# BioinformaticsArchive/HSA

Hardware: AMD Instinct MI355X
Metric: aligned reads/sec, 100bp synthetic vs hg19-sized 2BWT, at 1/2/4/8 MI355X (higher is better)
Workload: dtype u32

## Files before the change

hsa_amd/csrc/hsa_index.hip:

```cpp
#include <chrono>
#include <cstring>
#include <hip/hip_runtime.h>
#include <rocprim/rocprim.hpp>
#include <stdarg.h>
#include <stdio.h>
#include <stdlib.h>
#include <string.h>

#include "hsa_device.h"
#include "hsa_internal.h"
#include "hsa_trie.h"

static thread_local char g_err[1024] = "";
int g_waves_per_cu = 32;
int g_pool_entries = 0;
int g_batch_k = getenv("HSA_BATCH_K") ? atoi(getenv("HSA_BATCH_K")) : 32;
int g_batch_idle = getenv("HSA_BATCH_IDLE") ? atoi(getenv("HSA_BATCH_IDLE")) : 768;
int g_hit_cap = 64;

void hsa_set_error(const char *fmt, ...)
{
    va_list ap;
    va_start(ap, fmt);
    vsnprintf(g_err, sizeof g_err, fmt, ap);
    va_end(ap);
}

extern "C" const char *hsa_last_error(void) { return g_err; }
extern "C" void hsa_gpu_set_error_text(const char *msg) { hsa_set_error("%s", msg); }

extern "C" int hsa_device_count(void)
{
    int n = 0;
    if (hipGetDeviceCount(&n) != hipSuccess) return 0;
    return n;
}

extern "C" void hsa_free(void *p) { free(p); }

extern "C" int hsa_configure(int waves_per_cu, int pool_entries, int hit_cap)
{
    if (waves_per_cu > 0) g_waves_per_cu = waves_per_cu;
    if (pool_entries > 0) {
        if (pool_entries > 65535) { hsa_set_error("pool_entries > 65535"); return HSA_E_ARG; }
        g_pool_entries = pool_entries;
    } else if (pool_entries < 0) {
        g_pool_entries = 0;
    }
    if (hit_cap > 0) g_hit_cap = hit_cap;
    return 0;
}

static void hsa_log_alloc(const char *what, size_t bytes, std::chrono::steady_clock::time_point t0)
{
    const double ms = std::chrono::duration<double, std::milli>(std::chrono::steady_clock::now() - t0).count();
    if (ms > 5.0 && getenv("HSA_VERBOSE")) fprintf(stderr, "[hsa] %s: hipMalloc of %.2f GB took %.1f ms\n", what, bytes / 1e9, ms);
}

int hsa_realloc_device(void **out, void **old, size_t bytes)
{
    *out = nullptr;
    if (hipMalloc(out, bytes) != hipSuccess) {
        (void)hipGetLastError();
        *out = nullptr;
        (void)hipFree(*old);
        *old = nullptr;
        if (hipMalloc(out, bytes) != hipSuccess) {
            (void)hipGetLastError();
            *out = nullptr;
            hsa_set_error("hipMalloc(%zu) failed", bytes);
            return HSA_E_MEM;
        }
        return 0;
    }
    (void)hipFree(*old);
    *old = nullptr;
    return 0;
}

int hsa_grow(void **p, size_t *cap, size_t need)
{
    if (need <= *cap && *p) return 0;
    size_t n = need + need / 4 + 4096;
    const auto t0 = std::chrono::steady_clock::now();
    void *np = nullptr;
    *cap = 0;
    if (hsa_realloc_device(&np, p, n)) return HSA_E_MEM;
    *p = np;
    *cap = n;
    hsa_log_alloc("buffer", n, t0);
    return 0;
}

void hsa_scratch_free(SearchScratch &s)
{
    (void)hipFree(s.pool); (void)hipFree(s.nxt); (void)hipFree(s.hbuf);
    const size_t lb = s.link_bytes;
    s = SearchScratch();
    s.link_bytes = lb;
}

extern "C" int hsa_index_release_scratch(hsa_index_t *ix)
{
    if (!ix) { hsa_set_error("hsa_index_release_scratch: null handle"); return HSA_E_ARG; }
    (void)hipSetDevice(ix->device);
    HSA_HIP(hipStreamSynchronize(ix->stream));
    hsa_scratch_free(ix->main); hsa_scratch_free(ix->big); hsa_scratch_free(ix->huge);
    void **bufs[] = {&ix->d_pf, &ix->d_pf2, &ix->d_sp, &ix->d_any, &ix->d_any_aux, &ix->d_help, &ix->d_hp, &ix->d_rf,
                     &ix->d_ch, &ix->d_sm};
    size_t *caps[] = {&ix->d_pf_cap, &ix->d_pf2_cap, &ix->d_sp_cap, &ix->d_any_cap, &ix->d_any_aux_cap, &ix->d_help_cap,
                      &ix->d_hp_cap, &ix->d_rf_cap, &ix->d_ch_cap, &ix->d_sm_cap};
    for (int i = 0; i < 10; ++i) {
        if (*bufs[i]) (void)hipFree(*bufs[i]);
        *bufs[i] = nullptr;
        *caps[i] = 0;
    }
    return 0;
}

int hsa_scratch_reserve(SearchScratch &s, size_t lanes, size_t pcap, size_t hcap, size_t link_bytes)
{
    const size_t pe = lanes * pcap, he = lanes * hcap;
    auto fail = [&]() {
        hsa_set_error("scratch allocation failed (lanes %zu, pool %zu, hits %zu)", lanes, pcap, hcap);
        (void)hipGetLastError();
        hsa_scratch_free(s);
        return HSA_E_MEM;
    };
    if (!s.pool || pe > s.pool_entries || link_bytes != s.link_bytes) {
        const size_t npe = pe > s.pool_entries ? pe : s.pool_entries;
        const auto t0 = std::chrono::steady_clock::now();
        void *np = nullptr, *nn = nullptr;
        if (hsa_realloc_device(&np, (void **)&s.pool, npe * sizeof(uint4)) ||
            hsa_realloc_device(&nn, &s.nxt, npe * link_bytes)) {
            (void)hipFree(np);
            return fail();
        }
        s.pool = (uint4 *)np; s.nxt = nn;
        s.pool_entries = npe;
        s.link_bytes = link_bytes;
        hsa_log_alloc("search scratch pool", npe * (sizeof(uint4) + link_bytes), t0);
    }
    if (!s.hbuf || he > s.hit_entries) {
        const size_t nhe = he > s.hit_entries ? he : s.hit_entries;
        const auto t0 = std::chrono::steady_clock::now();
        void *nh = nullptr;
        if (hsa_realloc_device(&nh, (void **)&s.hbuf, nhe * 9 * sizeof(uint32_t))) return fail();
        s.hbuf = (uint32_t *)nh;
        s.hit_entries = nhe;
        hsa_log_alloc("search scratch hits", nhe * 9 * sizeof(uint32_t), t0);
    }
    return 0;
}

__global__ void k_msb_to_lsb(uint32_t *w, size_t n, uint32_t T)
{
    size_t i = (size_t)blockIdx.x * blockDim.x + threadIdx.x;
    if (i >= n) return;
    uint32_t x = w[i];
    x = (x >> 16) | (x << 16);
    x = ((x & 0xFF00FF00u) >> 8) | ((x & 0x00FF00FFu) << 8);
    x = ((x & 0xF0F0F0F0u) >> 4) | ((x & 0x0F0F0F0Fu) << 4);
    x = ((x & 0xCCCCCCCCu) >> 2) | ((x & 0x33333333u) << 2);
    if (i == n - 1 && (T & 15)) x &= (1u << (2 * (T & 15))) - 1u;
    w[i] = x;
}

struct U4 { uint32_t a, b, c, d; };
struct U4Plus {
    __host__ __device__ U4 operator()(const U4 &x, const U4 &y) const
    {
        return U4{x.a + y.a, x.b + y.b, x.c + y.c, x.d + y.d};
    }
};
// ... 704 lines not shown
```

hsa_amd/csrc/hsa_internal.h:

```cpp
#pragma once
#include <hip/hip_runtime.h>
#include <stdint.h>
#include <string>

#include "../../include/hsa_gpu.h"
#include "hsa_device.h"
#include "hsa_sa.h"

void hsa_set_error(const char *fmt, ...);

#define HSA_HIP(call)                                                                       \
    do {                                                                                    \
        hipError_t e_ = (call);                                                             \
        if (e_ != hipSuccess) {                                                             \
            hsa_set_error("%s:%d %s: %s", __FILE__, __LINE__, #call, hipGetErrorString(e_)); \
            return HSA_E_HIP;                                                               \
        }                                                                                   \
    } while (0)

enum : uint32_t {
    CTR_Q_MAIN = 0,
    CTR_HITS = 1,
    CTR_RANK = 2,
    CTR_SECTORS = 3,
    CTR_POPS = 4,
    CTR_ERRORS = 5,
    CTR_Q_FWD = 6,
    CTR_WIDTH_Q = 7,
    CTR_OVF_MAIN = 8,
    CTR_Q_BIG = 9,
    CTR_TRIE = 10,
    CTR_Q_MG = 10,
    CTR_UNFINISHED = 11,
    CTR_OVF_BIG = 12,
    CTR_FWD_Q_ALL = 13,
    CTR_FWD_Q_REF = 14,
    CTR_Q_HUGE = 15,
    CTR_SLOTS = 16
};

struct SearchScratch {
    size_t pool_entries = 0, hit_entries = 0;
    uint4 *pool = nullptr;
    void *nxt = nullptr;
    uint32_t *hbuf = nullptr;
    size_t link_bytes = 2;
};

struct hsa_index {
    int device = 0;
    uint32_t T = 0, isa0 = 0, C[5] = {0, 0, 0, 0, 0};
    uint32_t rT = 0, risa0 = 0, rC[5] = {0, 0, 0, 0, 0};
    uint4 *blk[2] = {nullptr, nullptr};
    void *blk_base[2] = {nullptr, nullptr};
    size_t nblk[2] = {0, 0};
    bool wide = false, is64 = false;
    uint64_t T64 = 0, isa0_64 = 0, C64[5] = {0, 0, 0, 0, 0};
    uint64_t rT64 = 0, risa0_64 = 0, rC64[5] = {0, 0, 0, 0, 0};
    bool any_wrap[2] = {false, false};
    hipStream_t stream = nullptr;
    int n_cu = 0;
    SearchScratch main, big, huge;
    void *d_ovf2 = nullptr; size_t d_ovf2_cap = 0;
    void *d_in = nullptr; size_t d_in_cap = 0;
    void *d_out = nullptr; size_t d_out_cap = 0;
    void *d_wrows = nullptr; size_t d_wrows_cap = 0;
    void *d_ovf = nullptr; size_t d_ovf_cap = 0;
    void *d_seed = nullptr; size_t d_seed_cap = 0;
    void *d_ext = nullptr; size_t d_ext_cap = 0;
    void *d_slices = nullptr; size_t d_slices_cap = 0;
    void *d_any = nullptr; size_t d_any_cap = 0;
    void *d_any_aux = nullptr; size_t d_any_aux_cap = 0;
    void *d_split = nullptr; size_t d_split_cap = 0;
    void *d_help = nullptr; size_t d_help_cap = 0;
    void *d_fwd = nullptr; size_t d_fwd_cap = 0;
    void *d_pf = nullptr; size_t d_pf_cap = 0;
    void *d_pf2 = nullptr; size_t d_pf2_cap = 0;
    void *h_pf = nullptr; size_t h_pf_cap = 0;
    uint32_t *d_sa = nullptr, *d_blocks = nullptr;
// ... 76 lines not shown
```

hsa_amd/csrc/hsa_search_kernels.h:

```cpp
#pragma once
#include <hip/hip_runtime.h>
#include <stdio.h>
#include <stdlib.h>
#include <string.h>

#include <type_traits>

#include "hsa_device.h"
#include "hsa_internal.h"
#include "hsa_trie.h"

#define NIL16 0xFFFFu
#define BLOCK 256
#define MAXB 128
#define MAXS 512

enum : uint32_t { PH_IDLE = 0, PH_POP, PH_EXACT, PH_EXPAND, PH_EXIT, PH_END, PH_WAIT };

struct SearchArgs {
    RankDir fwd, rev;
    uint32_t T;
    uint32_t C[5];
    RankDir64 fwd64, rev64;
    uint64_t T64;
// ... 41 lines not shown
    const int32_t *perm;
    uint32_t okey;
    int32_t *fwd_list;
    unsigned long long *fwd_n;
    uint32_t fwd_only;
    int32_t *rmap;
    uint32_t fr_budget, fr_demand, fr_cap;
    uint32_t *fr_ent;
    uint32_t *fr_tag;
    uint32_t *fr_rq;
    uint32_t *fr_st;
    unsigned long long *fr_q, *fr_p;
    unsigned long long *fr_c;
    const void *stw;
    uint32_t sdc;
};
#define FR_HIT 0x80000000u
#define FR_DONE 0x40000000u
#define FR_EW 8u
#define FR_CH 16u
#define FR_WALK 1024u
#ifndef HSA_HELPERS
#define HSA_HELPERS 1
#endif

typedef const __attribute__((address_space(4))) SearchArgs *ColdArgs;
__device__ __forceinline__ ColdArgs cold_args()
{
    ColdArgs p = (ColdArgs)(__builtin_amdgcn_kernarg_segment_ptr());
    asm volatile("" : "+s"(p));
    return p;
}

__device__ __forceinline__ uint32_t meta_pack(uint32_t i, uint32_t st, uint32_t isd, uint32_t mm, uint32_t go,
                                              uint32_t ge)
{
    return i | st << 10 | isd << 12 | mm << 13 | go << 20 | ge << 24;
}
#define M_I(m) ((int)((m) & 1023u))
#define M_ST(m) ((int)(((m) >> 10) & 3u))
#define M_ISD(m) ((int)(((m) >> 12) & 1u))
#define M_MM(m) ((int)(((m) >> 13) & 127u))
#define M_GO(m) ((int)(((m) >> 20) & 15u))
#define M_GE(m) ((int)((m) >> 24))

#define C_PH(c) ((c) & 7u)
#define C_STRAND(c) (((c) >> 3) & 1u)
#define C_SEED(c) (((c) >> 4) & 1u)
#define C_REG(c) (((c) >> 5) & 1u)
#define C_VT(c) (((c) >> 6) & 1u)
#define C_ALIAS(c) (((c) >> 7) & 1u)
#define C_OVF(c) (((c) >> 8) & 3u)
#define C_LEN(c) ((int)(((c) >> 10) & 1023u))
#define C_SLEN(c) ((int)(((c) >> 20) & 1023u))
#define SET_PH(c, p) ((c) = ((c) & ~7u) | (p))

template <typename V>
__device__ __forceinline__ V pick4(const V v[4], uint32_t c)
{
    return hsa_sel4<V>(c, v[0], v[1], v[2], v[3]);
}

template <typename IT> struct Ix;
template <> struct Ix<uint32_t> {
    __device__ static const RankDir &fwd(const SearchArgs &a) { return a.fwd; }
    __device__ static const RankDir &rev(const SearchArgs &a) { return a.rev; }
    __device__ static uint32_t T(const SearchArgs &a) { return a.T; }
    __device__ static const uint32_t *C(const SearchArgs &a) { return a.C; }
};
template <> struct Ix<uint64_t> {
    __device__ static const RankDir64 &fwd(const SearchArgs &a) { return a.fwd64; }
    __device__ static const RankDir64 &rev(const SearchArgs &a) { return a.rev64; }
    __device__ static uint64_t T(const SearchArgs &a) { return a.T64; }
    __device__ static const uint64_t *C(const SearchArgs &a) { return a.C64; }
};

template <typename IT> struct Ent {
    IT x, y, z;
    uint32_t w;
};
#ifndef HSA_WAVES_SIMD
#define HSA_WAVES_SIMD 4
#endif
#ifndef HSA_POOL_CHUNK
#define HSA_POOL_CHUNK 1
#endif
template <typename IT>
__device__ __forceinline__ size_t pool_base(size_t wv, uint32_t pcap, int lane)
{
#if HSA_POOL_CHUNK
    return (sizeof(IT) == 4 ? 1u : 2u) * wv * (size_t)((pcap + 31u) & ~31u) * 64 + (size_t)lane * 4;
#else
    return (sizeof(IT) == 4 ? 1u : 2u) * wv * pcap * 64 + (size_t)lane;
#endif
}
template <typename IT>
__device__ __forceinline__ size_t ent_at(size_t base, uint32_t slot)
{
#if HSA_POOL_CHUNK
    constexpr uint32_t EQ = sizeof(IT) == 4 ? 4u : 2u, U = sizeof(IT) == 4 ? 1u : 2u;
    return base + (size_t)(slot / EQ) * 256 + (slot % EQ) * U;
#else
    return base + (size_t)slot * (sizeof(IT) == 4 ? 64 : 128);
#endif
}
template <typename IT>
__device__ __forceinline__ Ent<IT> ent_load(const uint4 *pool, size_t base, uint32_t slot)
{
    const size_t i = ent_at<IT>(base, slot);
    if constexpr (sizeof(IT) == 4) {
        const uint4 v = pool[i];
        return Ent<IT>{v.x, v.y, v.z, v.w};
    } else {
        const uint4 u = pool[i], v = pool[i + (HSA_POOL_CHUNK ? 1 : 64)];
        return Ent<IT>{(uint64_t)u.x | (uint64_t)u.y << 32, (uint64_t)u.z | (uint64_t)u.w << 32,
                       (uint64_t)v.x | (uint64_t)v.y << 32, v.z};
    }
}
template <typename IT>
__device__ __forceinline__ void ent_store(uint4 *pool, size_t base, uint32_t slot, const Ent<IT> &e)
{
    const size_t i = ent_at<IT>(base, slot);
    if constexpr (sizeof(IT) == 4) {
        pool[i] = make_uint4(e.x, e.y, e.z, e.w);
    } else {
        pool[i] = make_uint4((uint32_t)e.x, (uint32_t)(e.x >> 32), (uint32_t)e.y, (uint32_t)(e.y >> 32));
        pool[i + (HSA_POOL_CHUNK ? 1 : 64)] = make_uint4((uint32_t)e.z, (uint32_t)(e.z >> 32), e.w, 0u);
    }
}
template <typename IT> struct HitW { static constexpr uint32_t STAGE = sizeof(IT) == 4 ? 9u : 10u;
                                     static constexpr uint32_t OUT = sizeof(IT) == 4 ? 9u : 14u; };

template <int MW> struct BMask;
template <> struct BMask<0> {
    uint32_t m0 = 0;
    __device__ __forceinline__ void clear() { m0 = 0; }
    __device__ __forceinline__ bool any() const { return m0 != 0; }
    __device__ __forceinline__ int lowest() const { return m0 ? __ffs(m0) - 1 : (1 << 30); }
    __device__ __forceinline__ bool test(int b) const { return (m0 >> b) & 1u; }
    __device__ __forceinline__ void set(int b) { m0 |= 1u << b; }
    __device__ __forceinline__ void reset(int b) { m0 &= ~(1u << b); }
};
template <> struct BMask<1> {
    uint64_t m0 = 0;
    __device__ __forceinline__ void clear() { m0 = 0; }
    __device__ __forceinline__ bool any() const { return m0 != 0; }
    __device__ __forceinline__ int lowest() const { return m0 ? __ffsll((unsigned long long)m0) - 1 : (1 << 30); }
    __device__ __forceinline__ bool test(int b) const { return (m0 >> b) & 1ull; }
    __device__ __forceinline__ void set(int b) { m0 |= 1ull << b; }
    __device__ __forceinline__ void reset(int b) { m0 &= ~(1ull << b); }
};
template <> struct BMask<2> {
    uint64_t m0 = 0, m1 = 0;
    __device__ __forceinline__ void clear() { m0 = m1 = 0; }
    __device__ __forceinline__ bool any() const { return (m0 | m1) != 0; }
    __device__ __forceinline__ int lowest() const
    {
        if (m0) return __ffsll((unsigned long long)m0) - 1;
        if (m1) return 64 + __ffsll((unsigned long long)m1) - 1;
        return 1 << 30;
// ... 336 lines not shown
            if (nf > 0) { na = nf; off = a.sp_off[2 * q + 1]; }
            else fl = HSA_F_FALLBACK;
        }
        a.n_aln[job] = na;
        a.flags[job] = fl;
        a.hit_off[job] = off;
    }
    for (int d = 32; d >= 1; d >>= 1) {
        q_add += __shfl_xor(q_add, d);
        p_add += __shfl_xor(p_add, d);
        w_add += __shfl_xor(w_add, d);
    }
    if ((threadIdx.x & 63) == 0) {
        if (q_add) atomicAdd(&a.ctr[CTR_RANK], q_add);
        if (p_add) atomicAdd(&a.ctr[CTR_POPS], p_add);
        if (w_add) { atomicAdd(&a.ctr[CTR_WIDTH_Q], w_add); atomicAdd(&a.ctr[CTR_FWD_Q_REF], w_add); }
    }
}

template <int MW, bool GAPS, typename WT, int NT, bool HUGE = false, typename IT = uint32_t, bool SN = false>
__global__ void __launch_bounds__(NT, HSA_WAVES_SIMD) k_search(SearchArgs a)
{
    using F = WFmt<WT>;
    using FS = SeedFmt<WT, SN>;
    static_assert(!SN || (std::is_same<WT, uint8_t>::value && !HUGE), "mixed format: 8-bit rows, not the HUGE pass");
    using E = Ent<IT>;
    using CT = typename std::conditional<sizeof(IT) == 8, int64_t, int>::type;
    constexpr uint32_t HW = HitW<IT>::STAGE, OW = HitW<IT>::OUT;
    const IT TT = Ix<IT>::T(a);
    const IT *const CC = Ix<IT>::C(a);
    using LT = typename std::conditional<HUGE, uint32_t, uint16_t>::type;
    constexpr bool FRH = !HUGE && HSA_HELPERS && GAPS && sizeof(IT) == 4 && !WFmt<WT>::NIB;
    constexpr uint32_t NIL = HUGE ? 0xFFFFFFFFu : (uint32_t)NIL16;
    constexpr bool IMP = !GAPS && !HUGE && sizeof(IT) == 4 && !WFmt<WT>::NIB;
#ifdef HSA_DIAG
    if (threadIdx.x == 0 && blockIdx.x < 8192) {
        g_diag[blockIdx.x * 4 + 0] = __builtin_amdgcn_s_memtime();
        g_diag[blockIdx.x * 4 + 1] = __builtin_amdgcn_s_memrealtime();
    }
#endif
    extern __shared__ __align__(16) uint8_t s_lds[];
    const uint32_t tid = threadIdx.x;
    const uint32_t gid = blockIdx.x * NT + tid;
    const int lane = (int)(tid & 63);
    for (uint32_t t = tid; t < 2 * a.ntab; t += NT) s_lds[t] = a.bmap[(t / a.ntab) * MAXS + t % a.ntab];
    static_assert(2 * sizeof(hsa_regime_t) <= 128, "regime LDS slot");
    hsa_regime_t *const s_reg = reinterpret_cast<hsa_regime_t *>(s_lds + 2 * a.ntab);
    if (tid < 2 * sizeof(hsa_regime_t) / 4)
        reinterpret_cast<uint32_t *>(s_reg)[tid] = reinterpret_cast<const uint32_t *>(a.regimes)[tid];
    __syncthreads();
    LT *const s_heads = reinterpret_cast<LT *>(s_lds + a.off_heads);
    using WTL = typename std::conditional<F::NIB, uint8_t, WT>::type;
    WTL *const s_wb = reinterpret_cast<WTL *>(s_lds + a.off_wb);
    WTL *const s_ws = reinterpret_cast<WTL *>(s_lds + a.off_ws);
    uint32_t *const s_nb = reinterpret_cast<uint32_t *>(s_lds + a.off_wb);
    uint32_t *const s_ns = reinterpret_cast<uint32_t *>(s_lds + a.off_ws);
    const size_t wv = gid >> 6;
#if HSA_POOL_CHUNK
    const size_t link0 = wv * (size_t)((a.pcap + 31u) & ~31u) * 64 + (size_t)lane * 32;
#define NXT(s) reinterpret_cast<LT *>(a.nxt)[link0 + (size_t)((s) >> 5) * 2048 + ((s) & 31u)]
#else
    const size_t link0 = wv * a.pcap * 64 + (size_t)lane;
#define NXT(s) reinterpret_cast<LT *>(a.nxt)[link0 + (size_t)(s) * 64]
#endif
    const size_t pbase = pool_base<IT>(wv, a.pcap, lane);
#define HB(i) r->hbuf[(wv * r->hcap * HW + (uint32_t)(i)) * 64 + lane]
// ... 52 lines not shown
            uint32_t &w = s_nb[((uint32_t)p >> 3) * NT + tid];
            const uint32_t sh = ((uint32_t)p & 7u) * 4u;
            w = (w & ~(15u << sh)) | v << sh;
        } else {
            WB(p) = (WTL)v;
        }
    };
    const uint8_t *rowp = nullptr;
    uint32_t cur_c = 0;
#ifndef HSA_ROWCACHE
#define HSA_ROWCACHE 1
#endif
    uint32_t rw_q = 0xFFFFFFFFu, rw_w = 0;
    auto getc = [&](int p) -> uint32_t {
        if constexpr (F::NIB && !HSA_ROWCACHE) {
            return WFmt<uint8_t>::code(rowp[((uint32_t)p >> 2) * 256u + ((uint32_t)p & 3u)]);
        } else if constexpr (F::NIB) {
            const uint32_t q = (uint32_t)p >> 2;
            if (q != rw_q) {
                rw_w = *reinterpret_cast<const uint32_t *>(rowp + q * 256u);
                rw_q = q;
            }
            return WFmt<uint8_t>::code((rw_w >> (((uint32_t)p & 3u) * 8u)) & 0xFFu);
        } else {
            return F::code(WB(p));
        }
    };
    auto bucket_of = [&](uint32_t m) -> int {
        if (!GAPS && a.mm_buckets) return M_MM(m);
        const int sc = SCORE(M_MM(m), M_GO(m), M_GE(m));
        return (uint32_t)sc < a.ntab ? (int)s_lds[C_REG(ctl) * a.ntab + sc] : 0xFF;
    };
    auto flush = [&](const E &v, int b) {
        if ((uint32_t)b >= a.nb) { ctl |= 1u << 8; return; }
        uint32_t slot;
        if (HUGE && free_head != NIL) {
            slot = free_head;
            free_head = NXT(slot);
        } else {
            if (pool_top >= a.pcap) { ctl |= 1u << 8; return; }
            slot = pool_top++;
        }
        DC(8);
        ent_store<IT>(a.pool, pbase, slot, v);
        const uint32_t old = mask.test(b) ? (uint32_t)HEAD(b) : NIL;
        NXT(slot) = (LT)old;
        HEAD(b) = (LT)slot;
        mask.set(b);
    };
    auto start_search = [&]() {
        best_score = SCORE(opt_max_diff + 1, R_MAXGO + 1, R_MAXGE + 1);
        max_diff = opt_max_diff;
        best_cnt = 0; n_aln = 0;
        mask.clear(); pool_top = 0; free_head = NIL;
        e = E{0, TT, 0, meta_pack((uint32_t)C_LEN(ctl), ST_M, 0, 0, 0, 0)};
        ctl |= 1u << 6;
        n_entries = 1;
        frs = 0; fr_p0 = st_p;
        SET_PH(ctl, PH_POP);
    };
    auto fr_key = [&]() -> uint32_t { return qpos * 2u + (1u - C_STRAND(ctl)); };
    auto row_base = [&](uint32_t cap_words) -> size_t {
        const int32_t *const rm = cold_args()->rmap;
        const uint32_t r = rm ? (C_STRAND(ctl) ? qpos : (uint32_t)rm[qpos]) : qpos * 2u + C_STRAND(ctl);
        return (size_t)(r >> 6) * cap_words * 64 + (r & 63u);
    };
// ... 479 lines not shown
                        const uint32_t sv = __hip_atomic_load(&r->fr_st[key], __ATOMIC_RELAXED, __HIP_MEMORY_SCOPE_AGENT);
                        if (frs & 2u) {
                            stop = (sv & (FR_HIT | FR_DONE)) != 0u;
                        } else if (sv == 0u && n_aln == 0) {
                            st_q = fr_q0 + (uint32_t)atomicAdd(&r->fr_q[key], 0ull);
                            st_p = fr_p0 + (uint32_t)atomicAdd(&r->fr_p[key], 0ull);
                            atomicAdd(&r->fr_c[7], 1ull);
                            stop = true;
                        }
                    }
                    const bool elig = !stop && !(frs & 5u) && n_aln == 0 && !C_OVF(ctl) && n_entries > 1 &&
                                      n_entries <= (int)FR_WALK && ps >= a.fr_budget && (fr_tick & 63u) == 0u;
                    const uint64_t em = __ballot(elig);
                    if (elig && lane == __ffsll((unsigned long long)em) - 1) {
                        const unsigned long long wt = __hip_atomic_load(&r->fr_c[3], __ATOMIC_RELAXED, __HIP_MEMORY_SCOPE_AGENT);
                        const unsigned long long rs = __hip_atomic_load(&r->fr_c[0], __ATOMIC_RELAXED, __HIP_MEMORY_SCOPE_AGENT);
                        const unsigned long long tk = __hip_atomic_load(&r->fr_c[1], __ATOMIC_RELAXED, __HIP_MEMORY_SCOPE_AGENT);
                        if (wt > rs - tk + a.fr_demand) {
                            if (!fr_offer()) frs |= 4u;
                            else if (frs & 2u) stop = true;
                            else { frs |= 1u; fr_p0 = st_p; fr_q0 = st_q; }
                        }
                    }
                    if (stop) { SET_PH(ctl, PH_END); continue; }
                }
            }
            if (C_VT(ctl)) {
                DC(3);
                ctl &= ~(1u << 6);
            } else {
                DC(4);
                const int b = mask.lowest();
                const uint32_t slot = HEAD(b);
                e = ent_load<IT>(a.pool, pbase, slot);
                const uint32_t nx = NXT(slot);
                if (nx == NIL) mask.reset(b);
                else HEAD(b) = (LT)nx;
                if (HUGE) { NXT(slot) = (LT)free_head; free_head = slot; }
            }
            --n_entries;
            ++st_p;
            const uint32_t m = e.w;
            if (!(R_MODE & MODE_NONSTOP) && SCORE(M_MM(m), M_GO(m), M_GE(m)) > best_score + S_MM) {
                SET_PH(ctl, PH_END);
                continue;
            }
            const int em = m_of(m);
            if (em < 0) { DC(18); continue; }
            const int ei = M_I(m);
            if (ei > 0 && em < (int)(wbg(ei - 1) & F::BIDM)) { DC(18); continue; }
            if (ei == 0) {
                DC(20);
                if (!on_hit(e.x, e.y, e.z, e.z + (e.y - e.x)) && !C_OVF(ctl)) SET_PH(ctl, PH_END);
                continue;
            }
            if (em == 0 && (M_ST(m) == ST_M || (R_MODE & MODE_GAPE) || M_GE(m) == R_MAXGE)) {
                ik = e.x; il = e.y; aux = e.z + (e.y - e.x); pos = (uint32_t)(ei - 1);
                SET_PH(ctl, PH_EXACT);
                continue;
            }
            req = 1; rp1 = e.x; rp2 = e.y + 1u;
            if constexpr (IMP) {
                const uint32_t len = (uint32_t)C_LEN(ctl), dp = len - (uint32_t)ei;
                if (len > a.sdc && dp < a.sdc) req = dp + 1u == a.sdc ? 2 : 4;
            }
            if constexpr (F::NIB) cur_c = getc(ei - 1);
            SET_PH(ctl, PH_EXPAND);
        } while (0);
// ... 156 lines not shown
                        const E v = entry((uint32_t)__ffs(rest) - 1u);
#ifdef HSA_DIAG
                        if (doomed(v.w)) DC(19);
#endif
                        flush(v, bucket_of(v.w));
                    }
                } else if (rest) {
                    const uint32_t g_go = (uint32_t)ego + (est == ST_M), g_ge = (uint32_t)ege + (est != ST_M);
                    const uint32_t mI = meta_pack((uint32_t)i, ST_I, 1u, (uint32_t)emm, g_go, g_ge);
                    const uint32_t mD = meta_pack((uint32_t)(i + 1), ST_D, 1u, (uint32_t)emm, g_go, g_ge);
                    const uint32_t mM = meta_pack((uint32_t)i, ST_M, 1u, (uint32_t)emm + 1u, (uint32_t)ego, (uint32_t)ege);
                    const uint32_t mP = meta_pack((uint32_t)i, ST_M, 0u, (uint32_t)emm, (uint32_t)ego, (uint32_t)ege);
                    const int bG = GAPS ? bucket_of(mI) : -1, bM = bucket_of(mM), bP = bucket_of(mP);
                    auto head0 = [&](int b) -> uint32_t {
                        return b >= 0 && (uint32_t)b < a.nb && mask.test(b) ? (uint32_t)HEAD(b) : NIL;
                    };
                    const uint32_t hG0 = GAPS ? head0(bG) : NIL, hM0 = head0(bM), hP0 = head0(bP);
                    uint32_t hG = hG0, hM = hM0, hP = hP0;
                    for (; rest; rest &= rest - 1u) {
                        const uint32_t b = (uint32_t)__ffs(rest) - 1u;
                        const bool ins = GAPS && b == 0, gap = GAPS && b <= 4u;
                        const bool mt = b == 8u && sc < 4;
                        const uint32_t c = gap ? b - 1u : (sc + b - 4u) & 3u;
                        IT k = pick4(oa, c), l = pick4(ob, c), rk = pick4(srk, c);
                        if (ins) { k = ek; l = el; rk = erk; }
                        const uint32_t meta = ins ? mI : gap ? mD : mt ? mP : mM;
                        const int bk = gap ? bG : mt ? bP : bM;
#ifdef HSA_DIAG
                        if (doomed(meta)) DC(19);
#endif
                        if ((uint32_t)bk >= a.nb || pool_top >= a.pcap) { ctl |= 1u << 8; continue; }
                        const uint32_t slot = pool_top++;
                        DC(8);
                        ent_store<IT>(a.pool, pbase, slot, E{k, l, rk, meta});
                        NXT(slot) = (LT)(bk == bG ? hG : bk == bM ? hM : hP);
                        hG = bk == bG ? slot : hG;
                        hM = bk == bM ? slot : hM;
                        hP = bk == bP ? slot : hP;
                    }
                    if (GAPS && hG != hG0) { HEAD(bG) = (LT)hG; mask.set(bG); }
                    if (hM != hM0) { HEAD(bM) = (LT)hM; mask.set(bM); }
                    if (hP != hP0) { HEAD(bP) = (LT)hP; mask.set(bP); }
                }
                const E v = entry(last);
#ifdef HSA_DIAG
                if (doomed(v.w)) DC(19);
#endif
                const int bk = bucket_of(v.w);
                if (bk <= mask.lowest()) { e = v; ctl |= 1u << 6; }
                else flush(v, bk);
            }
            SET_PH(ctl, PH_POP);
        }
#ifdef HSA_DIAG
        TMARK(3);
#endif
    }

#ifdef HSA_DIAG
    __syncthreads();
    if (threadIdx.x == 0 && blockIdx.x < 8192) {
        g_diag[blockIdx.x * 4 + 2] = __builtin_amdgcn_s_memtime();
        g_diag[blockIdx.x * 4 + 3] = __builtin_amdgcn_s_memrealtime();
    }
    for (int i = 0; i < 18; ++i)
        if (i < 9 || i > 12) atomicAdd(&g_dctr[i], (unsigned long long)dc[i]);
    for (int i = 18; i < 21; ++i) atomicAdd(&g_dctr[i], (unsigned long long)dc[i]);
    if (lane == 0)
// ... 43 lines not shown
```

hsa_amd/csrc/hsa_search_launch.h:

```cpp
#pragma once
#include <map>
#include <mutex>

#include "hsa_search_kernels.h"

static int check_regimes(const hsa_regime_t *rg, int n)
{
    for (int r = 0; r < n; ++r) {
        const hsa_regime_t &R = rg[r];
        if (R.s_mm < 0 || R.s_gapo < 0 || R.s_gape < 0) { hsa_set_error("negative penalty"); return HSA_E_ARG; }
        if (R.n_stacks <= 0 || R.n_stacks > ANY_MAX_STACKS) {
            hsa_set_error("n_stacks %d outside 1..%d", R.n_stacks, ANY_MAX_STACKS);
            return HSA_E_ARG;
        }
        if (R.max_gapo < 0 || R.max_gape < 0) { hsa_set_error("max_gapo/max_gape negative"); return HSA_E_ARG; }
        if (R.max_diff < -1) { hsa_set_error("max_diff out of range"); return HSA_E_ARG; }
    }
    return 0;
}

static int bucket_map(const hsa_regime_t &R, uint8_t map[MAXS])
{
    bool used[MAXS] = {false};
    const int md = R.max_diff < 0 ? 0 : R.max_diff;
// ... 70 lines not shown
    size_t lds;
    bool huge;
    uint32_t ntab;
    size_t resident;
    size_t res_lanes = 0;
};

enum { PASS_MAIN = 0, PASS_BIG = 1, PASS_HUGE = 2 };

using SearchFn = void (*)(SearchArgs);

template <typename WT, int NT, typename IT, bool SN>
static SearchFn search_kernel_nt(const LaunchPlan &P)
{
    if (P.nb <= 32) return P.gaps ? k_search<0, true, WT, NT, false, IT, SN> : k_search<0, false, WT, NT, false, IT, SN>;
    if (P.nb <= 64) return P.gaps ? k_search<1, true, WT, NT, false, IT, SN> : k_search<1, false, WT, NT, false, IT, SN>;
    return P.gaps ? k_search<2, true, WT, NT, false, IT, SN> : k_search<2, false, WT, NT, false, IT, SN>;
}

template <typename IT>
static SearchFn search_kernel(const LaunchPlan &P)
{
    if (P.nib)
        return P.nt == 64 ? search_kernel_nt<WNib, 64, IT, false>(P) : search_kernel_nt<WNib, 256, IT, false>(P);
    if (P.snib)
        return P.nt == 64 ? search_kernel_nt<uint8_t, 64, IT, true>(P) : search_kernel_nt<uint8_t, 256, IT, true>(P);
    if (P.huge) {
        if (P.wide) return P.gaps ? k_search<2, true, uint16_t, 64, true, IT> : k_search<2, false, uint16_t, 64, true, IT>;
        return P.gaps ? k_search<2, true, uint8_t, 64, true, IT> : k_search<2, false, uint8_t, 64, true, IT>;
    }
    if (P.wide) return P.nt == 64 ? search_kernel_nt<uint16_t, 64, IT, false>(P) : search_kernel_nt<uint16_t, 256, IT, false>(P);
    return P.nt == 64 ? search_kernel_nt<uint8_t, 64, IT, false>(P) : search_kernel_nt<uint8_t, 256, IT, false>(P);
}

static int kernel_waves_simd(SearchFn f)
{
    static std::mutex mu;
    static std::map<SearchFn, int> known;
    std::lock_guard<std::mutex> lock(mu);
    const auto it = known.find(f);
    if (it != known.end()) return it->second;
    int w = HSA_WAVES_SIMD;
    hipFuncAttributes at{};
    if (hipFuncGetAttributes(&at, reinterpret_cast<const void *>(f)) == hipSuccess && at.numRegs > 0) {
        w = 512 / ((at.numRegs + 7) / 8 * 8);
        w = w > 8 ? 8 : w < 1 ? 1 : w;
    } else {
        (void)hipGetLastError();
    }
    known[f] = w;
    return w;
}

template <typename IT = uint32_t>
static int plan_launch(hsa_index *ix, int n_jobs, int max_len, int max_seed, const RegimePlan &R, int mode,
                       LaunchPlan &P)
{
    constexpr uint32_t ent_bytes = 4u * sizeof(IT);
    const int nb = R.nb, max_entries = R.max_entries;
    const bool gaps = R.gaps, wide = R.wide, nib_ok = R.nib_ok;
    const bool big = mode == PASS_BIG;
    P.huge = mode == PASS_HUGE;
    P.ntab = (uint32_t)ix->staged_ntab;
    P.nb = (uint32_t)nb;
    P.gaps = gaps;
    P.wide = wide;
// ... 42 lines not shown
    if (nib_ok && !wide && !P.huge && !no_nib && !force_snib &&
        (force_nib || (!gaps && per_cu * (int)(P.nt / 64) < 16))) {
        const int waves8 = per_cu * (int)(P.nt / 64);
        const LaunchPlan keep = P;
        P.nib = true;
        P.snib = false;
        const int per_nib = best();
        if (!force_nib && per_nib * (int)(P.nt / 64) <= waves8) { P = keep; }
        else per_cu = per_nib;
    }
    if (P.lds > 160 * 1024) { hsa_set_error("reads too long for the LDS budget (%zu bytes)", P.lds); return HSA_E_ARG; }
    if (per_cu < 1) { hsa_set_error("search kernel does not fit (LDS %zu)", P.lds); return HSA_E_ARG; }
    const uint32_t NTB = P.nt;
    size_t blocks = (size_t)ix->n_cu * per_cu;
    P.resident = blocks * NTB;
    size_t need_blocks = ((size_t)n_jobs + NTB - 1) / NTB;
    if (P.huge) {
        blocks = 1;
    } else if (big) {
        static const size_t big_lanes = getenv("HSA_BIG_LANES") ? strtoull(getenv("HSA_BIG_LANES"), nullptr, 10) : 4096;
        const size_t big_blocks = big_lanes / NTB > 0 ? big_lanes / NTB : 1;
        blocks = need_blocks < big_blocks ? need_blocks : big_blocks;
        P.res_lanes = big_blocks * NTB;
    } else if (need_blocks < blocks) {
        blocks = need_blocks;
    }
    if (blocks < 1) blocks = 1;
    P.blocks = blocks;
    P.lanes = blocks * NTB;
    if (getenv("HSA_VERBOSE")) {
        int occ = 0;
        (void)hipOccupancyMaxActiveBlocksPerMultiprocessor(&occ, k_search<1, true, uint8_t, 256>, 256, P.lds);
        fprintf(stderr, "[hsa] launch: %d CUs x %d workgroups of %u lanes (runtime occupancy query says %d), "
                "LDS %zu B, %zu workgroups, %d buckets%s\n", ix->n_cu, per_cu, P.nt, occ, P.lds, blocks, nb,
                P.nib ? ", 4-bit rows" : P.snib ? ", 4-bit seed row" : "");
    }
    static const int pool_env = getenv("HSA_POOL_ENTRIES") ? atoi(getenv("HSA_POOL_ENTRIES")) : 0;
    const int pool_main = g_pool_entries ? g_pool_entries : pool_env > 0 && pool_env <= 65535 ? pool_env : 0;
    P.pcap = big ? 65535u : (uint32_t)(pool_main ? pool_main : (gaps ? (max_len <= 128 ? 16384 : 32768) : 8192));
    static const int pool_short = getenv("HSA_POOL_SHORT") ? atoi(getenv("HSA_POOL_SHORT")) : 8192;
    if (!big && !pool_main && max_len <= 32 && pool_short > 0 && pool_short <= 65535) P.pcap = (uint32_t)pool_short;
    P.hcap = big ? 16384u : (uint32_t)g_hit_cap;
    if (P.huge) {
        const uint64_t want = (uint64_t)(max_entries > 0 ? max_entries : 0) + 16u;
        P.pcap = (uint32_t)(want < (4ull << 20) ? want : (4ull << 20));
        P.hcap = 262144u;
    } else if (ent_bytes > 16 && !big) {
        const size_t budget = (size_t)64 << 30;
        if (P.lanes * P.pcap * ent_bytes > budget) {
            const size_t p = budget / (P.lanes * ent_bytes);
            P.pcap = (uint32_t)(p < 1024 ? 1024 : p);
        }
    }
    return 0;
}

template <typename IT>
static void launch_search(const LaunchPlan &P, const SearchArgs &A, hipStream_t st)
{
    hipLaunchKernelGGL(search_kernel<IT>(P), dim3((unsigned)P.blocks), dim3(P.nt), P.lds, st, A);
}

static uint32_t trie_levels(const hsa_index *ix, bool wide)
{
    const char *te = getenv("HSA_TRIE");
    return ix->trie_depth > 0 && ix->trie_wide == wide && !(te && atoi(te) == 0) ? ix->trie_depth : 0u;
}

// ... 92 lines not shown
    if (e) return atoi(e) != 0;
    return (help ? (size_t)io.n : 2 * (size_t)io.n) <= P.resident;
}

template <typename IT>
static int help_args(hsa_index *ix, SearchArgs &A, size_t items, const LaunchPlan &P, hipStream_t st)
{
    if (!help_kernel<IT>(P) || ix->staged_min_entries <= (int)P.pcap + 16) return 0;
    auto env = [](const char *k, long d) { const char *v = getenv(k); return v ? atol(v) : d; };
    const long budget = env("HSA_HELP_BUDGET", 512), demand = env("HSA_HELP_DEMAND", (long)(P.lanes / 2));
    const long cap = env("HSA_HELP_CAP", 1l << 20);
    if (budget <= 0 || cap <= 0 || cap > (1l << 24) || demand < 0 || items >= (1u << 26)) return 0;
    auto al = [](size_t x) { return (x + 255) / 256 * 256; };
    const size_t o_st = 256, o_q = o_st + al(items * 4), o_p = o_q + al(items * 8), o_tag = o_p + al(items * 8);
    const size_t o_rq = o_tag + al((size_t)cap * 4);
    const size_t o_ent = o_rq + al((size_t)cap * 4), total = o_ent + (size_t)cap * FR_CH * FR_EW * 4;
    int rc = hsa_grow(&ix->d_help, &ix->d_help_cap, total);
    if (rc) return rc;
    char *d = (char *)ix->d_help;
    HSA_HIP(hipMemsetAsync(d, 0, o_ent, st));
    A.fr_budget = (uint32_t)budget; A.fr_demand = (uint32_t)demand; A.fr_cap = (uint32_t)cap;
    A.fr_c = (unsigned long long *)d;
    A.fr_st = (uint32_t *)(d + o_st);
    A.fr_q = (unsigned long long *)(d + o_q);
    A.fr_p = (unsigned long long *)(d + o_p);
    A.fr_tag = (uint32_t *)(d + o_tag);
    A.fr_rq = (uint32_t *)(d + o_rq);
    A.fr_ent = (uint32_t *)(d + o_ent);
    return 0;
}

static int scratch_fit(hsa_index *ix, SearchScratch &S, LaunchPlan &P, size_t EW)
{
    const size_t lb = P.huge ? 4 : 2, floor_cap = 512;
    auto pe_of = [&](uint32_t pc) { return (size_t)((pc + 31u) & ~31u) * EW; };
    const size_t rl = P.res_lanes > P.lanes ? P.res_lanes : P.lanes;
    auto bytes = [&](uint32_t pc) { return rl * (pe_of(pc) * (16 + lb) + (size_t)P.hcap * EW * 36); };
    const bool held = S.pool && lb == S.link_bytes && rl * pe_of(P.pcap) <= S.pool_entries &&
                      rl * (size_t)P.hcap * EW <= S.hit_entries;
    if (!held && !P.huge) {
        const char *cm = getenv("HSA_SCRATCH_MB");
        const size_t cap_mb = cm ? strtoull(cm, nullptr, 10) : 0;
        size_t fr = 0, tot = 0;
        if (hipMemGetInfo(&fr, &tot) != hipSuccess) { (void)hipGetLastError(); fr = (size_t)-1 / 2; }
        fr += S.pool_entries * (16 + S.link_bytes) + S.hit_entries * 36;
        size_t avail = fr > ((size_t)2 << 30) ? fr - ((size_t)2 << 30) : 0;
        if (cap_mb && avail > (cap_mb << 20)) avail = cap_mb << 20;
        const uint32_t want = P.pcap;
        while (bytes(P.pcap) > avail && P.pcap > floor_cap) P.pcap = P.pcap / 2 > floor_cap ? P.pcap / 2 : floor_cap;
        if (P.pcap != want && getenv("HSA_VERBOSE"))
            fprintf(stderr, "[hsa] search scratch: pool %u -> %u entries per lane (%.1f GB for %zu lanes; %.1f GB "
                            "available)\n", want, P.pcap, bytes(P.pcap) / 1e9, P.lanes, avail / 1e9);
    }
    for (;;) {
        const int rc = hsa_scratch_reserve(S, rl, pe_of(P.pcap), (size_t)P.hcap * EW, lb);
        if (rc != HSA_E_MEM || P.huge || P.pcap <= floor_cap) return rc;
        P.pcap = P.pcap / 2 > floor_cap ? P.pcap / 2 : floor_cap;
        if (getenv("HSA_VERBOSE")) fprintf(stderr, "[hsa] search scratch: allocation failed, pool -> %u per lane\n", P.pcap);
    }
}

template <typename IT = uint32_t>
static int launch_pass(hsa_index *ix, const LaunchPlan &P0, SearchScratch &S, const PassIO &io, const PassLink &lk,
                       hipStream_t st)
{
    const int n = io.n;
    const bool mg = io.mg.d_mg != nullptr;
    const bool first = lk.qctr == CTR_Q_MAIN;
    const bool split = use_split(P0, io, lk, help_kernel<IT>(P0));
    LaunchPlan P = P0;
    if (split) {
        const size_t need = (2 * (size_t)n + P.nt - 1) / P.nt, cap = P.resident / P.nt;
        P.blocks = need < cap ? need : cap;
        P.lanes = P.blocks * P.nt;
    }
// ... 367 lines not shown
```

Before: 61.03 million.

## Store pool free-list links inside the entry word instead of a side array

For 32-bit non-gapped, non-wide searches and all 64-bit searches, the per-entry next link is packed into the spare bits of the entry's meta word (or into the unused fourth word of the second uint4). A push or pop then touches one memory location instead of two, removing the separate NXT array access. Host scratch sizing is reworked so link_bytes can be zero and existing allocations are reused when the link size grows. The packing depends on meta fields fitting into 16 bits, which static_asserts check.

```diff
diff --git a/hsa_amd/csrc/hsa_index.hip b/hsa_amd/csrc/hsa_index.hip
--- a/hsa_amd/csrc/hsa_index.hip
+++ b/hsa_amd/csrc/hsa_index.hip
@@ -54,7 +54,8 @@
 static void hsa_log_alloc(const char *what, size_t bytes, std::chrono::steady_clock::time_point t0)
 {
     const double ms = std::chrono::duration<double, std::milli>(std::chrono::steady_clock::now() - t0).count();
-    if (ms > 5.0 && getenv("HSA_VERBOSE")) fprintf(stderr, "[hsa] %s: hipMalloc of %.2f GB took %.1f ms\n", what, bytes / 1e9, ms);
+    const char *v = getenv("HSA_VERBOSE");
+    if (v && (ms > 5.0 || atoi(v) >= 2)) fprintf(stderr, "[hsa] %s: hipMalloc of %.2f GB took %.1f ms\n", what, bytes / 1e9, ms);
 }
 
 int hsa_realloc_device(void **out, void **old, size_t bytes)
@@ -95,9 +96,7 @@
 void hsa_scratch_free(SearchScratch &s)
 {
     (void)hipFree(s.pool); (void)hipFree(s.nxt); (void)hipFree(s.hbuf);
-    const size_t lb = s.link_bytes;
     s = SearchScratch();
-    s.link_bytes = lb;
 }
 
 extern "C" int hsa_index_release_scratch(hsa_index_t *ix)
@@ -127,19 +126,22 @@
         hsa_scratch_free(s);
         return HSA_E_MEM;
     };
-    if (!s.pool || pe > s.pool_entries || link_bytes != s.link_bytes) {
+    const size_t lbn = link_bytes > s.link_bytes ? link_bytes : s.link_bytes;
+    const bool grow = !s.pool || pe > s.pool_entries;
+    if (grow || lbn != s.link_bytes) {
         const size_t npe = pe > s.pool_entries ? pe : s.pool_entries;
         const auto t0 = std::chrono::steady_clock::now();
         void *np = nullptr, *nn = nullptr;
-        if (hsa_realloc_device(&np, (void **)&s.pool, npe * sizeof(uint4)) ||
-            hsa_realloc_device(&nn, &s.nxt, npe * link_bytes)) {
+        if ((grow && hsa_realloc_device(&np, (void **)&s.pool, npe * sizeof(uint4))) ||
+            (lbn && hsa_realloc_device(&nn, &s.nxt, npe * lbn))) {
             (void)hipFree(np);
             return fail();
         }
-        s.pool = (uint4 *)np; s.nxt = nn;
+        if (grow) s.pool = (uint4 *)np;
+        if (lbn) s.nxt = nn;
         s.pool_entries = npe;
-        s.link_bytes = link_bytes;
-        hsa_log_alloc("search scratch pool", npe * (sizeof(uint4) + link_bytes), t0);
+        s.link_bytes = lbn;
+        hsa_log_alloc("search scratch pool", npe * ((grow ? sizeof(uint4) : 0) + lbn), t0);
     }
     if (!s.hbuf || he > s.hit_entries) {
         const size_t nhe = he > s.hit_entries ? he : s.hit_entries;
diff --git a/hsa_amd/csrc/hsa_internal.h b/hsa_amd/csrc/hsa_internal.h
--- a/hsa_amd/csrc/hsa_internal.h
+++ b/hsa_amd/csrc/hsa_internal.h
@@ -44,7 +44,7 @@
     uint4 *pool = nullptr;
     void *nxt = nullptr;
     uint32_t *hbuf = nullptr;
-    size_t link_bytes = 2;
+    size_t link_bytes = 0;
 };
 
 struct hsa_index {
diff --git a/hsa_amd/csrc/hsa_search_kernels.h b/hsa_amd/csrc/hsa_search_kernels.h
--- a/hsa_amd/csrc/hsa_search_kernels.h
+++ b/hsa_amd/csrc/hsa_search_kernels.h
@@ -97,11 +97,30 @@
     return p;
 }
 
-__device__ __forceinline__ uint32_t meta_pack(uint32_t i, uint32_t st, uint32_t isd, uint32_t mm, uint32_t go,
-                                              uint32_t ge)
+constexpr __host__ __device__ __forceinline__ uint32_t meta_pack(uint32_t i, uint32_t st, uint32_t isd, uint32_t mm,
+                                                                 uint32_t go, uint32_t ge)
 {
     return i | st << 10 | isd << 12 | mm << 13 | go << 20 | ge << 24;
 }
+constexpr __host__ __device__ __forceinline__ uint32_t meta_link_pack(uint32_t m, uint32_t link)
+{
+    return (m & 1023u) | ((m >> 12) & 1u) << 10 | ((m >> 13) & 31u) << 11 | link << 16;
+}
+constexpr __host__ __device__ __forceinline__ uint32_t meta_link_meta(uint32_t w)
+{
+    return (w & 1023u) | ((w >> 10) & 1u) << 12 | ((w >> 11) & 31u) << 13;
+}
+constexpr __host__ __device__ __forceinline__ uint32_t meta_link_next(uint32_t w) { return w >> 16; }
+#define META_LINK_RT(i, isd, mm, link)                                                                      \
+    (meta_link_meta(meta_link_pack(meta_pack(i, ST_M, isd, mm, 0, 0), link)) == meta_pack(i, ST_M, isd, mm, 0, 0) && \
+     meta_link_next(meta_link_pack(meta_pack(i, ST_M, isd, mm, 0, 0), link)) == (link))
+static_assert(META_LINK_RT(1023u, 1u, 31u, 0u), "entry link: round trip at the field limits");
+static_assert(META_LINK_RT(1023u, 1u, 31u, 0xFFFEu), "entry link: round trip at the field limits");
+static_assert(META_LINK_RT(1023u, 1u, 31u, NIL16), "entry link: round trip at the field limits");
+static_assert(META_LINK_RT(0u, 0u, 0u, NIL16) && META_LINK_RT(0u, 0u, 0u, 0u), "entry link: round trip of zero fields");
+static_assert(META_LINK_RT(1023u, 0u, 0u, 0x8000u) && META_LINK_RT(0u, 1u, 0u, 0u) && META_LINK_RT(0u, 0u, 31u, 0u),
+              "entry link: each field alone");
+#undef META_LINK_RT
 #define M_I(m) ((int)((m) & 1023u))
 #define M_ST(m) ((int)(((m) >> 10) & 3u))
 #define M_ISD(m) ((int)(((m) >> 12) & 1u))
@@ -150,6 +169,13 @@
 #ifndef HSA_POOL_CHUNK
 #define HSA_POOL_CHUNK 1
 #endif
+#ifndef HSA_POOL_LINK
+#define HSA_POOL_LINK 1
+#endif
+constexpr __host__ __device__ bool pool_link_in_entry(bool huge, bool it64, bool gaps, bool rows16)
+{
+    return HSA_POOL_LINK && !huge && (it64 || (!gaps && !rows16));
+}
 template <typename IT>
 __device__ __forceinline__ size_t pool_base(size_t wv, uint32_t pcap, int lane)
 {
@@ -191,6 +217,32 @@
     } else {
         pool[i] = make_uint4((uint32_t)e.x, (uint32_t)(e.x >> 32), (uint32_t)e.y, (uint32_t)(e.y >> 32));
         pool[i + (HSA_POOL_CHUNK ? 1 : 64)] = make_uint4((uint32_t)e.z, (uint32_t)(e.z >> 32), e.w, 0u);
+    }
+}
+template <typename IT>
+__device__ __forceinline__ Ent<IT> ent_load_link(const uint4 *pool, size_t base, uint32_t slot, uint32_t &link)
+{
+    const size_t i = ent_at<IT>(base, slot);
+    if constexpr (sizeof(IT) == 4) {
+        const uint4 v = pool[i];
+        link = meta_link_next(v.w);
+        return Ent<IT>{v.x, v.y, v.z, meta_link_meta(v.w)};
+    } else {
+        const uint4 u = pool[i], v = pool[i + (HSA_POOL_CHUNK ? 1 : 64)];
+        link = v.w;
+        return Ent<IT>{(uint64_t)u.x | (uint64_t)u.y << 32, (uint64_t)u.z | (uint64_t)u.w << 32,
+                       (uint64_t)v.x | (uint64_t)v.y << 32, v.z};
+    }
+}
+template <typename IT>
+__device__ __forceinline__ void ent_store_link(uint4 *pool, size_t base, uint32_t slot, const Ent<IT> &e, uint32_t link)
+{
+    const size_t i = ent_at<IT>(base, slot);
+    if constexpr (sizeof(IT) == 4) {
+        pool[i] = make_uint4(e.x, e.y, e.z, meta_link_pack(e.w, link));
+    } else {
+        pool[i] = make_uint4((uint32_t)e.x, (uint32_t)(e.x >> 32), (uint32_t)e.y, (uint32_t)(e.y >> 32));
+        pool[i + (HSA_POOL_CHUNK ? 1 : 64)] = make_uint4((uint32_t)e.z, (uint32_t)(e.z >> 32), e.w, link);
     }
 }
 template <typename IT> struct HitW { static constexpr uint32_t STAGE = sizeof(IT) == 4 ? 9u : 10u;
@@ -593,6 +645,7 @@
     using LT = typename std::conditional<HUGE, uint32_t, uint16_t>::type;
     constexpr bool FRH = !HUGE && HSA_HELPERS && GAPS && sizeof(IT) == 4 && !WFmt<WT>::NIB;
     constexpr uint32_t NIL = HUGE ? 0xFFFFFFFFu : (uint32_t)NIL16;
+    constexpr bool LK = pool_link_in_entry(HUGE, sizeof(IT) == 8, GAPS, std::is_same<WT, uint16_t>::value);
     constexpr bool IMP = !GAPS && !HUGE && sizeof(IT) == 4 && !WFmt<WT>::NIB;
 #ifdef HSA_DIAG
     if (threadIdx.x == 0 && blockIdx.x < 8192) {
@@ -711,6 +764,19 @@
         return (uint32_t)sc < a.ntab ? (int)s_lds[C_REG(ctl) * a.ntab + sc] : 0xFF;
     };
     auto flush = [&](const E &v, int b) {
+        if constexpr (LK) {
+            uint32_t ovf = 1u;
+            if ((uint32_t)b < a.nb && pool_top < a.pcap) {
+                const uint32_t slot = pool_top++;
+                DC(8);
+                ent_store_link<IT>(a.pool, pbase, slot, v, mask.test(b) ? (uint32_t)HEAD(b) : NIL);
+                HEAD(b) = (LT)slot;
+                mask.set(b);
+                ovf = 0u;
+            }
+            ctl |= ovf << 8;
+            return;
+        }
         if ((uint32_t)b >= a.nb) { ctl |= 1u << 8; return; }
         uint32_t slot;
         if (HUGE && free_head != NIL) {
@@ -1256,8 +1322,13 @@
                 DC(4);
                 const int b = mask.lowest();
                 const uint32_t slot = HEAD(b);
-                e = ent_load<IT>(a.pool, pbase, slot);
-                const uint32_t nx = NXT(slot);
+                uint32_t nx;
+                if constexpr (LK) {
+                    e = ent_load_link<IT>(a.pool, pbase, slot, nx);
+                } else {
+                    e = ent_load<IT>(a.pool, pbase, slot);
+                    nx = NXT(slot);
+                }
                 if (nx == NIL) mask.reset(b);
                 else HEAD(b) = (LT)nx;
                 if (HUGE) { NXT(slot) = (LT)free_head; free_head = slot; }
@@ -1480,8 +1551,12 @@
                         if ((uint32_t)bk >= a.nb || pool_top >= a.pcap) { ctl |= 1u << 8; continue; }
                         const uint32_t slot = pool_top++;
                         DC(8);
-                        ent_store<IT>(a.pool, pbase, slot, E{k, l, rk, meta});
-                        NXT(slot) = (LT)(bk == bG ? hG : bk == bM ? hM : hP);
+                        if constexpr (LK) {
+                            ent_store_link<IT>(a.pool, pbase, slot, E{k, l, rk, meta}, bk == bG ? hG : bk == bM ? hM : hP);
+                        } else {
+                            ent_store<IT>(a.pool, pbase, slot, E{k, l, rk, meta});
+                            NXT(slot) = (LT)(bk == bG ? hG : bk == bM ? hM : hP);
+                        }
                         hG = bk == bG ? slot : hG;
                         hM = bk == bM ? slot : hM;
                         hP = bk == bP ? slot : hP;
diff --git a/hsa_amd/csrc/hsa_search_launch.h b/hsa_amd/csrc/hsa_search_launch.h
--- a/hsa_amd/csrc/hsa_search_launch.h
+++ b/hsa_amd/csrc/hsa_search_launch.h
@@ -126,6 +126,8 @@
     if (P.wide) return P.nt == 64 ? search_kernel_nt<uint16_t, 64, IT, false>(P) : search_kernel_nt<uint16_t, 256, IT, false>(P);
     return P.nt == 64 ? search_kernel_nt<uint8_t, 64, IT, false>(P) : search_kernel_nt<uint8_t, 256, IT, false>(P);
 }
+
+static bool plan_entry_links(const LaunchPlan &P, size_t EW) { return pool_link_in_entry(P.huge, EW == 2, P.gaps, P.wide); }
 
 static int kernel_waves_simd(SearchFn f)
 {
@@ -234,8 +236,9 @@
         int occ = 0;
         (void)hipOccupancyMaxActiveBlocksPerMultiprocessor(&occ, k_search<1, true, uint8_t, 256>, 256, P.lds);
         fprintf(stderr, "[hsa] launch: %d CUs x %d workgroups of %u lanes (runtime occupancy query says %d), "
-                "LDS %zu B, %zu workgroups, %d buckets%s\n", ix->n_cu, per_cu, P.nt, occ, P.lds, blocks, nb,
-                P.nib ? ", 4-bit rows" : P.snib ? ", 4-bit seed row" : "");
+                "LDS %zu B, %zu workgroups, %d buckets%s%s\n", ix->n_cu, per_cu, P.nt, occ, P.lds, blocks, nb,
+                P.nib ? ", 4-bit rows" : P.snib ? ", 4-bit seed row" : "",
+                plan_entry_links(P, sizeof(IT) / 4) ? ", links in the entries" : "");
     }
     static const int pool_env = getenv("HSA_POOL_ENTRIES") ? atoi(getenv("HSA_POOL_ENTRIES")) : 0;
     const int pool_main = g_pool_entries ? g_pool_entries : pool_env > 0 && pool_env <= 65535 ? pool_env : 0;
@@ -394,15 +397,24 @@
 
 static int scratch_fit(hsa_index *ix, SearchScratch &S, LaunchPlan &P, size_t EW)
 {
-    const size_t lb = P.huge ? 4 : 2, floor_cap = 512;
+    const size_t lb = P.huge ? 4 : plan_entry_links(P, EW) ? 0 : 2, floor_cap = 512;
+    const size_t lba = lb > S.link_bytes ? lb : S.link_bytes;
     auto pe_of = [&](uint32_t pc) { return (size_t)((pc + 31u) & ~31u) * EW; };
     const size_t rl = P.res_lanes > P.lanes ? P.res_lanes : P.lanes;
-    auto bytes = [&](uint32_t pc) { return rl * (pe_of(pc) * (16 + lb) + (size_t)P.hcap * EW * 36); };
-    const bool held = S.pool && lb == S.link_bytes && rl * pe_of(P.pcap) <= S.pool_entries &&
-                      rl * (size_t)P.hcap * EW <= S.hit_entries;
+    auto bytes = [&](uint32_t pc) { return rl * (pe_of(pc) * (16 + lba) + (size_t)P.hcap * EW * 36); };
+    const char *cm = getenv("HSA_SCRATCH_MB");
+    const size_t cap_mb = cm ? strtoull(cm, nullptr, 10) : 0;
+    const bool fits = S.pool && rl * pe_of(P.pcap) <= S.pool_entries && rl * (size_t)P.hcap * EW <= S.hit_entries;
+    bool held = fits && lb <= S.link_bytes;
+    if (fits && !held && !P.huge) {
+        size_t fr = 0, tot = 0;
+        if (hipMemGetInfo(&fr, &tot) != hipSuccess) { (void)hipGetLastError(); fr = (size_t)-1 / 2; }
+        const size_t need = S.pool_entries * lb + ((size_t)2 << 30);
+        const size_t all = S.pool_entries * (16 + lb) + S.hit_entries * 36;
+        if (need <= fr && !(cap_mb && all > (cap_mb << 20))) held = true;
+        else hsa_scratch_free(S);
+    }
     if (!held && !P.huge) {
-        const char *cm = getenv("HSA_SCRATCH_MB");
-        const size_t cap_mb = cm ? strtoull(cm, nullptr, 10) : 0;
         size_t fr = 0, tot = 0;
         if (hipMemGetInfo(&fr, &tot) != hipSuccess) { (void)hipGetLastError(); fr = (size_t)-1 / 2; }
         fr += S.pool_entries * (16 + S.link_bytes) + S.hit_entries * 36;
```

Measured after the change: 62.97 million, median of 6. 1.03x the previous value.
